# tanmayb123/OpenAI-Whisper-CoreML

Hardware: AMD Instinct MI355X
Metric: audio-sec/s (RTF) + decoder tok/s, Whisper-large-v2 30s chunks, 1->8 GPU (higher is better)
Workload: dtype bf16

## Files before the change

include/whisper_mi355x_debug.h:

```cpp
#ifndef WHISPER_MI355X_DEBUG_H
#define WHISPER_MI355X_DEBUG_H

#include "whisper_mi355x.h"

#ifdef __cplusplus
extern "C" {
#endif

WM_API int wmdbg_mel_filterbank(int n_mels, float *out);
WM_API int wmdbg_mel80(float *out);

WM_API int wmdbg_gemm(wm_ctx *ctx, const float *A, const float *W, const float *bias, float *C, int M, int N,
               int K, int epi);
WM_API int wmdbg_layernorm(wm_ctx *ctx, const float *x, const float *g, const float *b, int rows, int d,
                    float *out_f32, float *out_bf16_as_f32);
WM_API int wmdbg_enc_attention(wm_ctx *ctx, const float *q, const float *k, const float *v, int B, int H, int S,
                        float *out);
WM_API int wmdbg_dec_gemv(wm_ctx *ctx, const float *x, const float *ln_g, const float *ln_b, const float *W,
                   const float *bias, float *out, int B, int N, int K);
WM_API int wmdbg_dec_gemv_resid(wm_ctx *ctx, const float *x, const float *W, const float *bias, float *resid, float *copy_bf16,
                         float *stats, int B, int N, int K);
WM_API int wmdbg_dec_attention(wm_ctx *ctx, const float *q, const float *k, const float *v, int B, int H, int T,
                        int n_keys, int nsplit, float *out);
WM_API int wmdbg_dec_self_attention_off(wm_ctx *ctx, const float *q, const float *k, const float *v, int B, int H, int T,
                                        int pos, const int32_t *off, float *out);

WM_API int wmdbg_bench_dec_gemv(wm_ctx *ctx, int B, int N, int K, int ln, int resid, int n_mats, int iters,
                         int nw_override, float *avg_us);
WM_API int wmdbg_bench_dec_attention(wm_ctx *ctx, int B, int H, int T, int n_keys, int nsplit, int n_slices,
                              int iters, float *avg_us);

WM_API int wmdbg_bench_launch_floor(wm_ctx *ctx, int iters, int grid, float *eager_us, float *graph_us);

WM_API int wmdbg_bench_graph_branches(wm_ctx *ctx, int iters, int grid, int us_each, float *one_us, float *two_us);

WM_API int wmdbg_bench_gemm(wm_ctx *ctx, int M, int N, int K, int epi, int iters, int n_w, float *us);

WM_API int wmdbg_set_gemm_tile(int tile);

WM_API int wmdbg_lane_parts(int B, int lanes, int explicit_lanes, int n_text_state);
WM_API int wmdbg_cu_mask(int cu_lo, int cu_hi, uint32_t *mask8);

WM_API int wmdbg_set_precision(wm_ctx *ctx, int precision);

WM_API int wmdbg_set_tuning(const char *key, int value);
WM_API int wmdbg_group_count(int B, int lanes, int explicit_lanes);
WM_API int wmdbg_right_align(const int32_t *prompts, int stride, const int32_t *prompt_len, int b0, int Bg, int32_t *table_out,
                             int32_t *off_out);

WM_API int wmdbg_cand_groups(int B, int N, int lanes, int explicit_lanes, int32_t *b0_out, int32_t *cg_out);
WM_API int wmdbg_dec_attention_cand(wm_ctx *ctx, const float *q, const float *k, const float *v, int C, int N, int H, int T,
                                    int n_keys, const int32_t *live_rows, int n_live, float *out);
WM_API int wmdbg_dec_attention_cand_shared(wm_ctx *ctx, const float *q, const float *k, const float *v, int C, int N, int H,
                                           int T, int n_keys, const int32_t *live_rows, int n_live, float *out);

WM_API int wmdbg_sample_noise(wm_ctx *ctx, uint64_t seed, int chunk, int gi, int n0, int count, float *g);

WM_API int wmdbg_dtw(wm_ctx *ctx, const float *x, int B, const int32_t *N, const int32_t *M, int ld, int32_t *start_frame_out);
WM_API int wmdbg_align_capture(wm_ctx *ctx, float *matrix_out);
WM_API int wmdbg_align_matrix(wm_ctx *ctx, const float *q, const float *keys, int L, int H, int B, int Tq, int J,
                              const int32_t *hl, const int32_t *hh, int S, const int32_t *n_text, const int32_t *n_frames,
                              int medfilt_width, float qk_scale, float *x, float *col_stats);
WM_API int wmdbg_align_token_prob(wm_ctx *ctx, const float *logits, int B, int V, int ldo, const int32_t *tok, int eot,
                                  float *prob);

WM_API int wmdbg_beam_select(int N, int n_from, int32_t eot, int32_t pad, int room, const float *sum, const int32_t *list_n,
                             const int32_t *list_tok, const float *list_lp, int32_t *n_next, int32_t *src, int32_t *tok,
                             float *lp, float *new_sum, int32_t *n_fin, int32_t *fin_src, float *fin_lp, float *fin_sum);
WM_API double wmdbg_rank_score(double sum, int n_text, float length_penalty);
WM_API int wmdbg_beam_fill_order(int N, const float *sum, int32_t *order_out);
WM_API int wmdbg_beam_trace(wm_ctx *ctx, float *trace_out);
WM_API int wmdbg_beam_topk(wm_ctx *ctx, const float *logits, int rows, int V, int N, const int32_t *suppress, int n_suppress,
                           const int32_t *rng, int32_t ts_begin, int32_t *list_n, int32_t *list_tok, float *list_lp);
WM_API int wmdbg_beam_reorder(wm_ctx *ctx, uint16_t *cache, int L2, int rows, int H, int T, int N, int pos, int n_prompt,
                              const int32_t *src, const int32_t *wdone, int32_t *seq, float *logprob);

#ifdef __cplusplus
}
#endif
#endif
```

openai-whisper-coreml_amd/csrc/debug_hooks.cpp:

```cpp
#include <math.h>
#include <stdio.h>
#include <stdlib.h>
#include <string.h>

#include <algorithm>
#include <vector>

#include "../../include/whisper_mi355x_debug.h"
#include "beam.h"
#include "model.h"

int wm_gemm_set_tile_override(int tile);
extern "C" int wmdbg_set_gemm_tile(int tile) { return wm_gemm_set_tile_override(tile); }

extern "C" int wmdbg_set_tuning(const char *key, int value) {
    WM_REQUIRE(key, WM_ERR_INVALID, "wmdbg_set_tuning: null key");
    struct { const char *name; int *field; } table[] = {
        {"gemv_tn", &g_wm_tuning.gemv_tn}, {"gemv_nblk", &g_wm_tuning.gemv_nblk}, {"gemv_no_ppw2", &g_wm_tuning.gemv_no_ppw2}, {"gemv_ppw2_nblk", &g_wm_tuning.gemv_ppw2_nblk},
        {"prefetch_max_b", &g_wm_tuning.prefetch_max_b}, {"xattn_split_below", &g_wm_tuning.xattn_split_below},
        {"xattn_wgs", &g_wm_tuning.xattn_wgs}, {"xattn_no_flat", &g_wm_tuning.xattn_no_flat},
        {"xattn_lds_pad", &g_wm_tuning.xattn_lds_pad}, {"xattn_splits", &g_wm_tuning.xattn_splits},
        {"gemm_tile", &g_wm_tuning.gemm_tile}, {"gemm128_pipe", &g_wm_tuning.gemm128_pipe}, {"gemm_gm", &g_wm_tuning.gemm_gm}, {"no_early_stop", &g_wm_tuning.no_early_stop},
        {"xattn_no_deep", &g_wm_tuning.xattn_no_deep}, {"xattn_never_short", &g_wm_tuning.xattn_never_short},         {"logits_tn", &g_wm_tuning.logits_tn}, {"enc_attn_mfma_sum", &g_wm_tuning.enc_attn_mfma_sum},
        {"group_chunks", &g_wm_tuning.group_chunks}, {"argmax_rows_per_wg", &g_wm_tuning.argmax_rows_per_wg}, {"xattn_fuse_q", &g_wm_tuning.xattn_fuse_q},
        {"lane_parts", &g_wm_tuning.lane_parts}, {"lane_solo_cus", &g_wm_tuning.lane_solo_cus}, {"frontend_per_wave_twiddles", &g_wm_tuning.frontend_per_wave_twiddles},
    };
    if (strcmp(key, "reset") == 0) { g_wm_tuning = WmTuning(); return WM_OK; }
    for (auto &e : table)
        if (strcmp(key, e.name) == 0) { *e.field = value; return WM_OK; }
    wm_set_error("wmdbg_set_tuning: unknown key '%s'", key);
    return WM_ERR_INVALID;
}

extern "C" int wmdbg_group_count(int B, int lanes, int explicit_lanes) { return wm_group_count(B, lanes, explicit_lanes != 0, 0); }
extern "C" int wmdbg_cand_groups(int B, int N, int lanes, int explicit_lanes, int32_t *b0_out, int32_t *cg_out) {
    if (B < 1 || N < 1 || N > WM_MAX_BEST_OF || !b0_out || !cg_out) return -1;
    std::vector<int> b0, cg;
    const int G = wm_cand_groups(B, N, lanes, explicit_lanes != 0, b0, cg);
    for (int g = 0; g < G; ++g) { b0_out[g] = b0[g]; cg_out[g] = cg[g]; }
    return G;
}
extern "C" int wmdbg_right_align(const int32_t *prompts, int stride, const int32_t *prompt_len, int b0, int Bg,
                                 int32_t *table_out, int32_t *off_out) {
    std::vector<int32_t> table, off;
    const int P = wm_right_align(prompts, stride, prompt_len, b0, Bg, table, off);
    std::copy(table.begin(), table.end(), table_out);
    std::copy(off.begin(), off.end(), off_out);
    return P;
}
extern "C" int wmdbg_lane_parts(int B, int lanes, int explicit_lanes, int n_text_state) {
    return wm_lane_parts(B, lanes, explicit_lanes != 0, n_text_state, 0);
}
extern "C" int wmdbg_cu_mask(int cu_lo, int cu_hi, uint32_t *mask8) { return wm_cu_mask(cu_lo, cu_hi, mask8); }

extern "C" int wmdbg_mel_filterbank(int n_mels, float *out) {
    WM_REQUIRE(out && n_mels > 0 && n_mels <= 256, WM_ERR_INVALID, "bad args");
    std::vector<float> f;
    wm_mel_filterbank(n_mels, f);
    memcpy(out, f.data(), f.size() * sizeof(float));
    return WM_OK;
}
extern "C" int wmdbg_mel80(float *out) {
    WM_REQUIRE(out, WM_ERR_INVALID, "null");
    memcpy(out, wm_mel80_table(), sizeof(float) * 80 * 201);
    return WM_OK;
}

static int up(void **d, const void *h, size_t bytes, hipStream_t s) {
    WM_HIP(hipMalloc(d, bytes + 512));
    WM_HIP(hipMemsetAsync(*d, 0, bytes + 512, s));
    if (h) WM_HIP(hipMemcpyAsync(*d, h, bytes, hipMemcpyHostToDevice, s));
    return WM_OK;
}
static void to_bf16(const float *in, std::vector<bf16_t> &out, size_t n) {
    out.resize(n);
    for (size_t i = 0; i < n; ++i) {
        uint32_t u;
        memcpy(&u, &in[i], 4);
        u += 0x7fffu + ((u >> 16) & 1u);
        out[i] = (bf16_t)(u >> 16);
    }
}
static void from_bf16(const std::vector<bf16_t> &in, float *out) {
    for (size_t i = 0; i < in.size(); ++i) {
        uint32_t u = (uint32_t)in[i] << 16;
        memcpy(&out[i], &u, 4);
    }
}

extern "C" int wmdbg_gemm(wm_ctx *ctx, const float *A, const float *W, const float *bias, float *C, int M, int N,
                          int K, int epi) {
    WM_TRY(wm_ctx_make_current(ctx));
    WM_REQUIRE(epi == EPI_F32 || epi == EPI_BIAS_BF16 || epi == EPI_GELU_BF16 || epi == EPI_RESID_F32, WM_ERR_INVALID,
               "wmdbg_gemm: epilogue %d not exposed", epi);
    std::vector<bf16_t> a16, w16;
    to_bf16(A, a16, (size_t)M * K);
    to_bf16(W, w16, (size_t)N * K);
    void *dA, *dW, *dB = nullptr, *dC;
    hipStream_t s = ctx->stream;
    WM_TRY(up(&dA, a16.data(), a16.size() * 2, s));
    WM_TRY(up(&dW, w16.data(), w16.size() * 2, s));
    if (bias) WM_TRY(up(&dB, bias, (size_t)N * 4, s));
    const bool f32out = (epi == EPI_F32 || epi == EPI_RESID_F32);
    WM_TRY(up(&dC, epi == EPI_RESID_F32 ? C : nullptr, (size_t)M * N * (f32out ? 4 : 2), s));
    GemmArgs g;
    memset(&g, 0, sizeof(g));
// ... 213 lines not shown
    to_bf16(v, v16, (size_t)B * H * T * 64);
    void *dq, *dk, *dv, *dp;
    hipStream_t s = ctx->stream;
    WM_TRY(up(&dq, q, (size_t)B * H * 64 * 4, s));
    WM_TRY(up(&dk, k16.data(), k16.size() * 2, s));
    WM_TRY(up(&dv, v16.data(), v16.size() * 2, s));
    WM_TRY(up(&dp, nullptr, (size_t)B * H * WM_MAXSPLIT * 66 * 4, s));
    void *datt;
    WM_TRY(up(&datt, nullptr, ((size_t)B + 15) / 16 * 16 * H * 64 * 2, s));
    int rc = nsplit == 0 ? wm_dec_self_attention(ctx, (const float *)dq, (const bf16_t *)dk, (const bf16_t *)dv, B, H, T,
                                                 n_keys, nullptr, (bf16_t *)datt)
                         : wm_dec_attention(ctx, (const float *)dq, (const bf16_t *)dk, (const bf16_t *)dv, B, H, T, n_keys,
                                            nullptr, nsplit < 0 ? 1 : nsplit, (float *)dp, (bf16_t *)datt, nsplit < 0);
    if (rc == WM_OK) {
        const size_t Bpad = ((size_t)B + 15) / 16 * 16, dd = (size_t)H * 64;
        std::vector<bf16_t> o16(Bpad * dd), lin((size_t)B * dd);
        WM_HIP(hipMemcpyAsync(o16.data(), datt, o16.size() * 2, hipMemcpyDeviceToHost, s));
        WM_HIP(hipStreamSynchronize(s));
        for (size_t b = 0; b < (size_t)B; ++b)
            for (size_t k = 0; k < dd; ++k) lin[b * dd + k] = o16[wm_tiled_offset(b, k, dd)];
        from_bf16(lin, out);
    }
    (void)hipFree(datt);
    (void)hipFree(dq); (void)hipFree(dk); (void)hipFree(dv); (void)hipFree(dp);
    return rc;
}

static int dec_attention_cand(wm_ctx *ctx, const float *q, const float *k, const float *v, int C, int N, int H, int T, int n_keys,
                              const int32_t *live_rows, int n_live, float *out, bool short_lived) {
    WM_TRY(wm_ctx_make_current(ctx));
    WM_REQUIRE(q && k && v && out, WM_ERR_INVALID, "dec_attention_cand: null pointer");
    WM_REQUIRE(N >= 1 && N <= WM_MAX_BEST_OF && C >= 1 && C * N <= WM_DEC_MAXB && H >= 1 && H <= 255 && T >= 1 && n_keys >= 1 &&
                   n_keys <= T,
               WM_ERR_INVALID, "dec_attention_cand: bad geometry");
    const int B = C * N;
    std::vector<int32_t> live((size_t)WM_DEC_MAXB + 4, 0);
    if (live_rows) {
        WM_REQUIRE(n_live >= 0 && n_live <= B, WM_ERR_INVALID, "dec_attention_cand: n_live %d outside [0, %d]", n_live, B);
        for (int i = 0; i < n_live; ++i) {
            WM_REQUIRE(live_rows[i] >= 0 && live_rows[i] < B && (i == 0 || live_rows[i] > live_rows[i - 1]), WM_ERR_INVALID,
                       "dec_attention_cand: the live list must be ascending rows of the group");
            live[i] = live_rows[i];
        }
        live[WM_DEC_MAXB] = n_live;
    }
    std::vector<bf16_t> k16, v16;
    to_bf16(k, k16, (size_t)C * H * T * 64);
    to_bf16(v, v16, (size_t)C * H * T * 64);
    void *dq, *dk, *dv, *dp, *dl, *datt;
    hipStream_t s = ctx->stream;
    const size_t att_b = ((size_t)B + 15) / 16 * 16 * H * 64 * 2;
    WM_TRY(up(&dq, q, (size_t)B * H * 64 * 4, s));
    WM_TRY(up(&dk, k16.data(), k16.size() * 2, s));
    WM_TRY(up(&dv, v16.data(), v16.size() * 2, s));
    WM_TRY(up(&dp, nullptr, (size_t)B * H * WM_MAXSPLIT * 66 * 4, s));
    WM_TRY(up(&dl, live.data(), live.size() * 4, s));
    WM_TRY(up(&datt, nullptr, att_b, s));
    WM_HIP(hipMemsetAsync(dp, 0, (size_t)B * H * WM_MAXSPLIT * 66 * 4, s));
    WM_HIP(hipMemsetAsync(datt, 0, att_b, s));
    const int *lr = live_rows ? (const int *)dl : nullptr;
    int rc = wm_dec_attention_cand(ctx, (const float *)dq, (const bf16_t *)dk, (const bf16_t *)dv, C, N, H, T, n_keys, (float *)dp,
                                   (bf16_t *)datt, nullptr, 0, 0, lr, lr ? lr + WM_DEC_MAXB : nullptr, short_lived);
    if (rc == WM_OK) {
        const size_t Bpad = ((size_t)B + 15) / 16 * 16, dd = (size_t)H * 64;
        std::vector<bf16_t> o16(Bpad * dd), lin((size_t)B * dd);
        WM_HIP(hipMemcpyAsync(o16.data(), datt, o16.size() * 2, hipMemcpyDeviceToHost, s));
        WM_HIP(hipStreamSynchronize(s));
        for (size_t b = 0; b < (size_t)B; ++b)
            for (size_t kk = 0; kk < dd; ++kk) lin[b * dd + kk] = o16[wm_tiled_offset(b, kk, dd)];
        from_bf16(lin, out);
    }
    void *fr[] = {dq, dk, dv, dp, dl, datt};
    for (void *p : fr) (void)hipFree(p);
    return rc;
}

extern "C" int wmdbg_dec_attention_cand(wm_ctx *ctx, const float *q, const float *k, const float *v, int C, int N, int H, int T,
                                        int n_keys, const int32_t *live_rows, int n_live, float *out) {
    return dec_attention_cand(ctx, q, k, v, C, N, H, T, n_keys, live_rows, n_live, out, false);
}
extern "C" int wmdbg_dec_attention_cand_shared(wm_ctx *ctx, const float *q, const float *k, const float *v, int C, int N, int H,
                                               int T, int n_keys, const int32_t *live_rows, int n_live, float *out) {
    return dec_attention_cand(ctx, q, k, v, C, N, H, T, n_keys, live_rows, n_live, out, true);
}

extern "C" int wmdbg_dec_self_attention_off(wm_ctx *ctx, const float *q, const float *k, const float *v, int B, int H, int T,
                                            int pos, const int32_t *off, float *out) {
    WM_TRY(wm_ctx_make_current(ctx));
    WM_REQUIRE(q && k && v && off && out, WM_ERR_INVALID, "dec_self_attention_off: null pointer");
    WM_REQUIRE(B >= 1 && B <= WM_DEC_MAXB && T >= 1 && pos >= 0 && pos < T, WM_ERR_INVALID, "dec_self_attention_off: bad geometry");
    for (int b = 0; b < B; ++b)
        WM_REQUIRE(off[b] >= 0 && off[b] < T, WM_ERR_INVALID, "dec_self_attention_off: off[%d] = %d outside [0, %d)", b, off[b], T);
    std::vector<bf16_t> k16, v16;
    to_bf16(k, k16, (size_t)B * H * T * 64);
    to_bf16(v, v16, (size_t)B * H * T * 64);
    void *dq, *dk, *dv, *doff, *dpos, *datt;
    hipStream_t s = ctx->stream;
    WM_TRY(up(&dq, q, (size_t)B * H * 64 * 4, s));
    WM_TRY(up(&dk, k16.data(), k16.size() * 2, s));
    WM_TRY(up(&dv, v16.data(), v16.size() * 2, s));
    WM_TRY(up(&doff, off, (size_t)B * 4, s));
    WM_TRY(up(&dpos, &pos, 4, s));
    WM_TRY(up(&datt, nullptr, ((size_t)B + 15) / 16 * 16 * H * 64 * 2, s));
    int rc = wm_dec_self_attention(ctx, (const float *)dq, (const bf16_t *)dk, (const bf16_t *)dv, B, H, T, 0, (const int *)dpos,
                                   (bf16_t *)datt, nullptr, 0, 0, nullptr, nullptr, (const int *)doff);
    if (rc == WM_OK) {
        const size_t Bpad = ((size_t)B + 15) / 16 * 16, dd = (size_t)H * 64;
        std::vector<bf16_t> o16(Bpad * dd), lin((size_t)B * dd);
        WM_HIP(hipMemcpyAsync(o16.data(), datt, o16.size() * 2, hipMemcpyDeviceToHost, s));
        WM_HIP(hipStreamSynchronize(s));
        for (size_t b = 0; b < (size_t)B; ++b)
            for (size_t j = 0; j < dd; ++j) lin[b * dd + j] = o16[wm_tiled_offset(b, j, dd)];
        from_bf16(lin, out);
    }
    void *fr[] = {dq, dk, dv, doff, dpos, datt};
    for (void *p : fr)
        if (p) (void)hipFree(p);
    return rc;
}


extern "C" int wmdbg_bench_dec_gemv(wm_ctx *ctx, int B, int N, int K, int ln, int resid, int n_mats, int iters,
                                    int nw_override, float *avg_us) {
    (void)nw_override;
    WM_TRY(wm_ctx_make_current(ctx));
    WM_REQUIRE(B >= 1 && B <= WM_DEC_MAXB, WM_ERR_INVALID, "wmdbg_bench_dec_gemv: B out of range");
    hipStream_t s = ctx->stream;
    const int Npad = ((N + 15) / 16) * 16;
    void *dW, *dx16, *dc, *dout, *dout16;
    WM_TRY(up(&dW, nullptr, (size_t)n_mats * Npad * K * 2, s));
    WM_TRY(up(&dx16, nullptr, (size_t)WM_DEC_MAXB * K * 2, s));
    WM_TRY(up(&dc, nullptr, (size_t)Npad * 4, s));
    WM_TRY(up(&dout, nullptr, (size_t)WM_DEC_MAXB * Npad * 4, s));
    WM_TRY(up(&dout16, nullptr, (size_t)WM_DEC_MAXB * Npad * 2, s));
    WM_HIP(hipMemsetAsync(dW, 0x3c, (size_t)n_mats * Npad * K * 2, s));
    DecGemvArgs a;
    memset(&a, 0, sizeof(a));
    a.B = B; a.N = N; a.K = K; a.out_f32 = (float *)dout; a.ldo = Npad; a.epi = resid ? DE_RESID : DE_Q;
    a.a = (const bf16_t *)dx16; a.c2 = (const float *)dc;
    void *dstat;
    WM_TRY(up(&dstat, nullptr, (size_t)(WM_DEC_MAXB / 16) * 2 * (K > N ? K : N) * 4 + 4096, s));
    if (resid) { a.stats_out = (float *)dstat; a.out_bf16 = (bf16_t *)dout16; }
    if (ln) { a.c1 = (const float *)dc; a.stats_in = (const float *)dstat; a.stats_parts = K / 16; }
    hipEvent_t e0, e1;
    WM_HIP(hipEventCreate(&e0));
    WM_HIP(hipEventCreate(&e1));
    int rc = WM_OK;
    hipGraph_t g = nullptr;
    hipGraphExec_t ge = nullptr;
    WM_HIP(hipStreamBeginCapture(s, hipStreamCaptureModeThreadLocal));
    for (int i = 0; i < iters && rc == WM_OK; ++i) {
        a.W = (const bf16_t *)dW + (size_t)(i % n_mats) * Npad * K;
        rc = wm_dec_gemv(ctx, a);
    }
    WM_HIP(hipStreamEndCapture(s, &g));
    if (rc == WM_OK) {
        WM_HIP(hipGraphInstantiate(&ge, g, nullptr, nullptr, 0));
        WM_HIP(hipGraphLaunch(ge, s));
        WM_HIP(hipStreamSynchronize(s));
        WM_HIP(hipEventRecord(e0, s));
        WM_HIP(hipGraphLaunch(ge, s));
    }
    WM_HIP(hipEventRecord(e1, s));
    WM_HIP(hipStreamSynchronize(s));
    float ms = 0.f;
    WM_HIP(hipEventElapsedTime(&ms, e0, e1));
// ... 445 lines not shown
```

openai-whisper-coreml_amd/csrc/dec_kernels.hip:

```cpp
#include <stdlib.h>

#include <atomic>
#include <string.h>

#include "dec_close.h"
#include "model.h"
#include "philox.h"

namespace {

typedef __attribute__((ext_vector_type(8))) __bf16 bf16x8;
typedef __attribute__((ext_vector_type(4))) float f32x4;
typedef __attribute__((ext_vector_type(4))) unsigned u32x4;

typedef __attribute__((ext_vector_type(2))) float f32x2;
typedef __attribute__((ext_vector_type(2))) __bf16 bf16x2;

__device__ __forceinline__ unsigned pack2(float a, float b) {
    const f32x2 v = {a, b};
    return __builtin_bit_cast(unsigned, __builtin_convertvector(v, bf16x2));
}
__device__ __forceinline__ float gelu_erf(float x) {
    return 0.5f * x * (1.0f + erff(x * 0.70710678118654752440f));
}
// ... 750 lines not shown
                    vb -= (long)(ob - pos_k) * 64;
                    ob = pos_k;
                    load_block(kb, vb, 0, 0, kall[0], vall[0]);
                }
            }
        }
        int nk = n_keys;
        if constexpr (OFF) nk = pos_k + 1 - ob;
        float qe[8];
#pragma unroll
        for (int i = 0; i < 4; ++i) {
            qe[i] = q0[i] * 0.125f;
            qe[4 + i] = q1[i] * 0.125f;
        }
        float m_run = -1e30f, l_run = 0.f;
        float oa[8] = {0, 0, 0, 0, 0, 0, 0, 0};
        auto process_block = [&](int r0, const u32x4 (&kv)[U], const u32x4 (&vv)[U]) {
            attn_block<NS, U, SELF>(qe, r0, stream, rg, nk, kv, vv, m_run, l_run, oa);
        };
        if (DEEP) {
#pragma unroll
            for (int blk = 0; blk < NB; ++blk)
                if (blk * (NS * 8 * U) < nk) process_block(blk * (NS * 8 * U), kall[blk], vall[blk]);
        } else {
            if (SPEC) {
                attn_block_fence<U>(kall[0], vall[0]);
                process_block(0, kall[0], vall[0]);
            }
            for (int r0 = SPEC ? NS * 8 * U : 0; r0 < nk; r0 += NS * 8 * U) {
                u32x4 kv[U], vv[U];
                load_block(kb, vb, r0, nk - 1, kv, vv);
                attn_block_fence<U>(kv, vv);
                process_block(r0, kv, vv);
            }
        }
        attn_stream_reduce(l_run, oa);
        if (nsplit > 1) {
            if (rg == 0) {
                float *po = cold.part + ((long)bh * NS + stream) * 66;
#pragma unroll
                for (int i = 0; i < 8; ++i) po[2 + e8 * 8 + i] = oa[i];
                if (e8 == 0) {
                    po[0] = m_run;
                    po[1] = l_run;
                }
            }
            continue;
        }
        if (rg == 0) {
#pragma unroll
            for (int i = 0; i < 8; ++i) wo_[wave][e8 * 8 + i] = oa[i];
            if (e8 == 0) {
                wm_[wave] = m_run;
                wl_[wave] = l_run;
            }
        }
        __syncthreads();
        if (tid < 64)
            cold.att[wm_tiled_offset((size_t)b, (size_t)(h * 64 + tid), (size_t)d)] = f2bf(attn_merge<NS>(wm_, wl_, &wo_[0][0], 64, tid));
    }
}

template <int NS, int U, bool NT, bool DEEP = false>
__global__ __launch_bounds__(DEEP ? 256 : NS * 64) void dec_xrows_attn_kernel(
    const float *__restrict__ q, const bf16_t *__restrict__ kc, const bf16_t *__restrict__ vc,
    const int *__restrict__ pos_ptr, const int *__restrict__ live_rows ,
    unsigned packA , unsigned packB ,
    unsigned packC , AttnCold cold) {
    const int H = (int)(packA & 0xffu), nsplit = (int)((packA >> 8) & 0xffu), flat_wpw = (int)(packA >> 16);
    const int T_stride = (int)(packB & 0xffffu), n_keys_const = (int)(packB >> 16);
    int n_bh = (int)(packC & 0xffffu);
    const int n_wg = (int)(packC >> 16);
    const int d = H * 64;
    const int *n_live_ptr = live_rows ? live_rows + WM_DEC_MAXB : nullptr;
    bf16_t *att = cold.att;
    float *part = cold.part;
    const char *pf_ptr = cold.pf_ptr;
    const long pf_tile_bytes = cold.pf_tile_bytes;
    if ((int)blockIdx.x >= n_wg) {
        l2_warm_tile(pf_ptr, pf_tile_bytes, (int)blockIdx.x - n_wg, blockDim.x);
        return;
    }
    if (n_live_ptr) n_bh = *n_live_ptr * H;
    __shared__ float wm_[NS], wl_[NS];
    __shared__ float wo_[NS][64];
    const int tid = threadIdx.x, lane = tid & 63, wave = tid >> 6;
    const int rg = lane >> 3, e8 = lane & 7;
    const int n_keys = pos_ptr ? (*pos_ptr + 1) : n_keys_const;
    const int last = n_keys - 1;
    int stream = (int)blockIdx.y * (NS / nsplit) + wave;
    int bh0 = blockIdx.x, bh_step = n_wg;
    if (flat_wpw > 0) {
        const int unit = (int)blockIdx.x * flat_wpw + wave;
        if (unit >= n_bh * NS) return;
        bh0 = unit / NS;
        stream = unit % NS;
        bh_step = n_bh;
    }
    for (int pi = bh0; pi < n_bh; pi += bh_step) {
        if (flat_wpw == 0 && pi != (int)blockIdx.x) __syncthreads();
        const int h = pi % H;
        const int b = live_rows ? live_rows[pi / H] : pi / H;
        const int bh = b * H + h;
        const bf16_t *kb = kc + (long)bh * T_stride * 64 + e8 * 8;
        const bf16_t *vb = vc + (long)bh * T_stride * 64 + e8 * 8;
        float qe[8];
        {
            const float *qp = q + (long)b * d + h * 64 + e8 * 8;
#pragma unroll
            for (int i = 0; i < 8; ++i) qe[i] = qp[i] * 0.125f;
        }
        float m_run = -1e30f, l_run = 0.f;
        float oa[8] = {0, 0, 0, 0, 0, 0, 0, 0};
        auto load_block = [&](int r0, u32x4 (&kv)[U], u32x4 (&vv)[U]) {
            attn_load_block<NS, U, NT>(kb, vb, r0, stream, rg, n_keys, last, kv, vv);
        };
        auto process_block = [&](int r0, const u32x4 (&kv)[U], const u32x4 (&vv)[U]) {
            attn_block<NS, U, false>(qe, r0, stream, rg, n_keys, kv, vv, m_run, l_run, oa);
        };
        if (DEEP) {
            constexpr int NB = ATT_MAXK / (NS * 8 * U);
            u32x4 kall[NB][U], vall[NB][U];
#pragma unroll
            for (int blk = 0; blk < NB; ++blk) load_block(blk * (NS * 8 * U), kall[blk], vall[blk]);
#pragma unroll
            for (int blk = 0; blk < NB; ++blk)
                if (blk * (NS * 8 * U) < n_keys) process_block(blk * (NS * 8 * U), kall[blk], vall[blk]);
        } else {
            for (int r0 = 0; r0 < n_keys; r0 += NS * 8 * U) {
                u32x4 kv[U], vv[U];
                load_block(r0, kv, vv);
                process_block(r0, kv, vv);
            }
        }
        attn_stream_reduce(l_run, oa);
        if (nsplit > 1) {
            if (rg == 0) {
                float *po = part + ((long)bh * NS + stream) * 66;
#pragma unroll
                for (int i = 0; i < 8; ++i) po[2 + e8 * 8 + i] = oa[i];
                if (e8 == 0) {
                    po[0] = m_run;
                    po[1] = l_run;
                }
            }
            continue;
        }
        if (rg == 0) {
#pragma unroll
            for (int i = 0; i < 8; ++i) wo_[wave][e8 * 8 + i] = oa[i];
            if (e8 == 0) {
                wm_[wave] = m_run;
                wl_[wave] = l_run;
            }
        }
        __syncthreads();
        if (tid < 64)
            att[wm_tiled_offset((size_t)b, (size_t)(h * 64 + tid), (size_t)d)] = f2bf(attn_merge<NS>(wm_, wl_, &wo_[0][0], 64, tid));
    }
}

struct CandLive {
    int r_lo, r_hi;
    unsigned long long head_lo, head_hi;
};
template <int N>
__device__ __forceinline__ void cand_window(const CandLive &L, int wj, int lane, int &c, unsigned &lm) {
    const int rank_lo = (int)__builtin_amdgcn_mbcnt_hi((unsigned)(L.head_lo >> 32), __builtin_amdgcn_mbcnt_lo((unsigned)L.head_lo, 0u));
    const int rank_hi = (int)__builtin_amdgcn_mbcnt_hi((unsigned)(L.head_hi >> 32), __builtin_amdgcn_mbcnt_lo((unsigned)L.head_hi, 0u)) +
                        __popcll(L.head_lo);
    const unsigned long long sel_lo = __ballot(((L.head_lo >> lane) & 1ull) && rank_lo == wj);
    const unsigned long long sel_hi = __ballot(((L.head_hi >> lane) & 1ull) && rank_hi == wj);
    int row;
    if (sel_lo) row = __builtin_amdgcn_readlane(L.r_lo, __builtin_ctzll(sel_lo));
    else row = __builtin_amdgcn_readlane(L.r_hi, sel_hi ? __builtin_ctzll(sel_hi) : 0);
    c = row / N;
    lm = 0u;
#pragma unroll
    for (int s = 0; s < N; ++s) {
        const int r = c * N + s;
        if ((__ballot(L.r_lo == r) | __ballot(L.r_hi == r)) != 0ull) lm |= 1u << s;
    }
}

template <int N, bool NT>
__global__ __launch_bounds__(512) void dec_xcand_attn_kernel(
    const float *__restrict__ q, const bf16_t *__restrict__ kc, const bf16_t *__restrict__ vc,
    const int *__restrict__ live_rows , bf16_t *__restrict__ att,
    float *__restrict__ part, unsigned packA , unsigned packB ,
    unsigned packC , const char *pf_ptr, long pf_tile_bytes) {
    constexpr int NS = 8, U = 4;
    static_assert(N >= 1 && N <= 8, "1 .. 8 candidates per window");
    constexpr int NP = N <= 5 ? N : (N + 1) / 2;
    const int H = (int)(packA & 0xffu), flat_wpw = (int)(packA >> 16);
    const int T_stride = (int)(packB & 0xffffu), n_keys = (int)(packB >> 16);
    const int C = (int)(packC & 0xffffu), n_wg = (int)(packC >> 16);
    const int d = H * 64;
    if ((int)blockIdx.x >= n_wg) {
        l2_warm_tile(pf_ptr, pf_tile_bytes, (int)blockIdx.x - n_wg, blockDim.x);
        return;
    }
    __shared__ float wm_[N][NS], wl_[N][NS];
    __shared__ float wo_[N][NS][64];
    const int tid = threadIdx.x, lane = tid & 63, wave = tid >> 6;
    const int rg = lane >> 3, e8 = lane & 7;
    const int last = n_keys - 1;
    CandLive L;
    {
        int n_live = C * N, p_lo = lane - 1, p_hi = lane + 63;
        L.r_lo = lane;
        L.r_hi = lane + 64;
        if (live_rows) {
            n_live = live_rows[WM_DEC_MAXB];
            L.r_lo = live_rows[lane];
            L.r_hi = live_rows[lane + 64];
            p_lo = live_rows[lane > 0 ? lane - 1 : 0];
            p_hi = live_rows[lane + 63];
        }
        const bool v_lo = lane < n_live, v_hi = lane + 64 < n_live;
        L.r_lo = v_lo ? L.r_lo : -1;
        L.r_hi = v_hi ? L.r_hi : -1;
        L.head_lo = __ballot(v_lo && (lane == 0 || p_lo / N != L.r_lo / N));
        L.head_hi = __ballot(v_hi && p_hi / N != L.r_hi / N);
    }
    const int n_pairs = (__popcll(L.head_lo) + __popcll(L.head_hi)) * H;
    int stream = wave;
    int p0 = blockIdx.x, p_step = n_wg;
    if (flat_wpw > 0) {
        const int unit = (int)blockIdx.x * flat_wpw + wave;
        if (unit >= n_pairs * NS) return;
        p0 = unit / NS;
        stream = unit % NS;
        p_step = n_pairs;
    }
    for (int pi = p0; pi < n_pairs; pi += p_step) {
        if (flat_wpw == 0 && pi != (int)blockIdx.x) __syncthreads();
        const int h = pi % H;
        int c;
        unsigned lm;
        cand_window<N>(L, pi / H, lane, c, lm);
        const int ch = c * H + h;
// ... 584 lines not shown
        if (two) {
            nblk = 2;
            p.bgroups = (blocks + 1) / 2;
        }
    }
    p.n_tg = (p.n_tiles + tn - 1) / tn;
    p.n_tg_pad = p.bgroups > 1 ? (p.n_tg + 7) / 8 * 8 : p.n_tg;
    int grid = p.n_tg_pad * p.bgroups;
    if (pf_enabled(a.B) && a.pf_ptr && a.pf_rows >= 16 && grid % 8 == 0) {
        p.pf_ptr = (const char *)a.pf_ptr;
        p.pf_tile_bytes = 16L * a.pf_k * 2;
        p.pf_tiles = a.pf_rows / 16;
        p.pf_head_major = a.pf_head_major;
        grid += a.pf_head_major ? 32 * (a.pf_head_major / a.B + 2) : p.pf_tiles;
    }
    switch (a.epi * 2 + (ln ? 1 : 0)) {
        case DE_QKV * 2 + 1: {
            WmProfScope ps(&ctx->prof, "dec_gemv_ln_qkv", ctx->stream);
            return launch_gemv<DE_QKV, true>(ctx, p, spw, tn, nblk, nw, grid, ppw);
        }
        case DE_Q * 2 + 1: {
            WmProfScope ps(&ctx->prof, "dec_gemv_ln_q", ctx->stream);
            return launch_gemv<DE_Q, true>(ctx, p, spw, tn, nblk, nw, grid, ppw);
        }
        case DE_GELU * 2 + 1: {
            WmProfScope ps(&ctx->prof, "dec_gemv_ln_fc1", ctx->stream);
            return launch_gemv<DE_GELU, true>(ctx, p, spw, tn, nblk, nw, grid, ppw);
        }
        case DE_LOGITS * 2 + 1: {
            WmProfScope ps(&ctx->prof, "dec_gemv_ln_logits", ctx->stream);
            return launch_gemv<DE_LOGITS, true>(ctx, p, spw, tn, nblk, nw, grid, ppw);
        }
        case DE_LOGITS_X * 2 + 1: {
            WmProfScope ps(&ctx->prof, "dec_gemv_ln_logits_x", ctx->stream);
            return launch_gemv<DE_LOGITS_X, true>(ctx, p, spw, tn, nblk, nw, grid, ppw);
        }
        case DE_RESID * 2: {
            WmProfScope ps(&ctx->prof, a.K > a.N ? "dec_gemv_fc2" : "dec_gemv_attn_out", ctx->stream);
            return launch_gemv<DE_RESID, false>(ctx, p, spw, tn, nblk, nw, grid, ppw);
        }
        case DE_Q * 2: {
            WmProfScope ps(&ctx->prof, "dec_gemv_plain", ctx->stream);
            return launch_gemv<DE_Q, false>(ctx, p, spw, tn, nblk, nw, grid, ppw);
        }
        default:
            wm_set_error("dec_gemv: unsupported (epilogue %d, LayerNorm %d) pair", a.epi, (int)ln);
            return WM_ERR_INVALID;
    }
}

int wm_ln_fold(wm_ctx *ctx, const bf16_t *W, const float *g, const float *beta, const float *bias, int N, int K,
               bf16_t *Wf, float *c1, float *c2) {
    const int npad = (N + 15) / 16 * 16;
    ln_fold_kernel<<<npad, 256, 0, ctx->stream>>>(W, g, beta, bias, N, K, Wf, c1, c2);
    WM_HIP(hipGetLastError());
    return WM_OK;
}

int wm_dec_embed(wm_ctx *ctx, const int *seq, const int *pos_ptr, int B, const bf16_t *emb, const float *pemb,
                 int d, float *x, bf16_t *xb, float *stats_out, float *mean_buf, const int *off) {
    WmProfScope ps(&ctx->prof, "dec_embed", ctx->stream);
    dec_embed_kernel<<<B, 256, 0, ctx->stream>>>(seq, pos_ptr, B, emb, pemb, d, x, xb, stats_out, mean_buf, off);
    WM_HIP(hipGetLastError());
    return WM_OK;
}

int wm_dec_attn_splits(int B, int H) {
    const int bh = B * H;
    const int thr = g_wm_tuning.xattn_split_below;
    if (bh >= thr) return 1;
    int ns = 2;
    while (ns < 8 && bh * ns < 192) ns *= 2;
    return ns;
}

int wm_dec_attention(wm_ctx *ctx, const float *q, const bf16_t *kc, const bf16_t *vc, int B, int H,
                     int T_stride, int n_keys, const int *pos_ptr, int nsplit, float *part, bf16_t *att,
                     bool cross, const bf16_t *pf_ptr, int pf_rows, int pf_k, const int *live_rows, const int *n_live,
                     bool short_lived) {
    WM_REQUIRE(nsplit == 1 || nsplit == 2 || nsplit == 4 || nsplit == 8, WM_ERR_INVALID,
               "dec_attention: nsplit %d is not 1, 2, 4 or 8", nsplit);
    WM_REQUIRE(T_stride <= ATT_MAXK && n_keys <= ATT_MAXK, WM_ERR_INVALID,
               "dec_attention: more than %d keys", ATT_MAXK);
    WM_REQUIRE(nsplit == 1 || part != nullptr, WM_ERR_INVALID, "dec_attention: split launch without a partials buffer");
    WM_REQUIRE(H >= 1 && H <= 255 && B * H < 65536, WM_ERR_INVALID, "dec_attention: %d heads x %d rows do not fit the packed arguments", H, B);
    WM_REQUIRE((!live_rows && !n_live) || n_live == live_rows + WM_DEC_MAXB, WM_ERR_INVALID, "dec_attention: the live count must follow the live rows");
    {
        WmProfScope ps(&ctx->prof, cross ? "dec_attn_cross" : "dec_attn_self", ctx->stream);
        const int cap_cus = g_wm_tuning.xattn_wgs > 0 && g_wm_tuning.xattn_wgs < ctx->n_cus ? g_wm_tuning.xattn_wgs : ctx->n_cus;
        const int cap = short_lived ? (1 << 30) : cap_cus;
        int n_wg = B * H;
        if (n_wg > cap) {
            const int rounds = (n_wg + cap - 1) / cap;
            n_wg = (n_wg + rounds - 1) / rounds;
        }
        int gx = n_wg;
        long tile_bytes = 0;
        if (pf_enabled(B) && pf_ptr && nsplit == 1 && gx % 8 == 0 && pf_rows >= 16) {
            tile_bytes = 16L * pf_k * 2;
            gx += pf_rows / 16;
        }
        const bool no_flat = g_wm_tuning.xattn_no_flat != 0;
        if (nsplit > 1 && !no_flat) {
            const int units = B * H * 8;
            int wpw = (units + 255) / 256;
            wpw = wpw < 1 ? 1 : (wpw > 4 ? 4 : wpw);
            const int g = (units + wpw - 1) / wpw;
            const AttnCold cold = {att, part, nullptr, 0};
            const unsigned pA = (unsigned)H | (8u << 8) | ((unsigned)wpw << 16), pB = (unsigned)T_stride | ((unsigned)n_keys << 16);
            const unsigned pC = (unsigned)(B * H) | ((unsigned)g << 16);
            WM_REQUIRE(g < 65536, WM_ERR_INVALID, "dec_attention: flat grid too large");
            if (g_wm_tuning.xattn_no_deep)
                dec_xrows_attn_kernel<8, 4, WM_XATTN_NT><<<g, wpw * 64, 0, ctx->stream>>>(
                    q, kc, vc, pos_ptr, live_rows, pA, pB, pC, cold);
            else if ((size_t)B * H * T_stride * 64 * 2 * 2 <= (size_t)3200 * 1024)
                dec_rows_attn_kernel<8, 4, false, true><<<g, wpw * 64, 0, ctx->stream>>>(
                    q, kc, vc, pos_ptr, live_rows, pA, pB, pC, cold);
            else
                dec_rows_attn_kernel<8, 4, WM_XATTN_NT, true><<<g, wpw * 64, 0, ctx->stream>>>(
                    q, kc, vc, pos_ptr, live_rows, pA, pB, pC, cold);
        } else {
            dim3 grid(gx, nsplit);
            const int lds_pad = g_wm_tuning.xattn_lds_pad;
            static std::atomic<int> pad_set[64];
            if (lds_pad > pad_set[ctx->device & 63].load(std::memory_order_acquire)) {
                WM_HIP(hipFuncSetAttribute((const void *)dec_xrows_attn_kernel<8, 4, WM_XATTN_NT>,
                                           hipFuncAttributeMaxDynamicSharedMemorySize, lds_pad));
                pad_set[ctx->device & 63].store(lds_pad, std::memory_order_release);
            }
            const AttnCold cold = {att, part, (const char *)pf_ptr, tile_bytes};
            const unsigned pA = (unsigned)H | ((unsigned)nsplit << 8), pB = (unsigned)T_stride | ((unsigned)n_keys << 16);
            const unsigned pC = (unsigned)(B * H) | ((unsigned)n_wg << 16);
            dec_xrows_attn_kernel<8, 4, WM_XATTN_NT><<<grid, (8 / nsplit) * 64, nsplit == 1 ? lds_pad : 0, ctx->stream>>>(
                q, kc, vc, pos_ptr, live_rows, pA, pB, pC, cold);
        }
        WM_HIP(hipGetLastError());
    }
    if (nsplit > 1) {
        WmProfScope ps(&ctx->prof, "dec_attn_combine", ctx->stream);
        dec_attn_combine_kernel<8><<<B * H, 64, 0, ctx->stream>>>(part, H, H * 64, att);
        WM_HIP(hipGetLastError());
    }
    return WM_OK;
}

namespace {
template <int N>
int launch_xcand(wm_ctx *ctx, const float *q, const bf16_t *kc, const bf16_t *vc, int C, int H, int T_stride, int n_keys,
                 float *part, bf16_t *att, const bf16_t *pf_ptr, int pf_rows, int pf_k, const int *live_rows, bool short_lived,
                 bool *flat) {
    const int pairs = C * H;
    *flat = pairs < 256 && !short_lived;
    const unsigned pB = (unsigned)T_stride | ((unsigned)n_keys << 16);
    long tile_bytes = 0;
    int warm = 0;
    if (pf_enabled(C * N) && pf_ptr && pf_rows >= 16) {
        tile_bytes = 16L * pf_k * 2;
        warm = pf_rows / 16;
    }
    if (*flat) {
        const int units = pairs * 8;
        int wpw = (units + 255) / 256;
        wpw = wpw < 1 ? 1 : (wpw > 8 ? 8 : wpw);
        const int g = (units + wpw - 1) / wpw;
        if (g % 8 != 0) warm = 0;
        const unsigned pA = (unsigned)H | ((unsigned)wpw << 16), pC = (unsigned)C | ((unsigned)g << 16);
        dec_xcand_attn_kernel<N, WM_XATTN_NT><<<g + warm, wpw * 64, 0, ctx->stream>>>(
            q, kc, vc, live_rows, att, part, pA, pB, pC, warm ? (const char *)pf_ptr : nullptr, warm ? tile_bytes : 0);
        WM_HIP(hipGetLastError());
        return WM_OK;
    }
    const int cap_cus = g_wm_tuning.xattn_wgs > 0 && g_wm_tuning.xattn_wgs < ctx->n_cus ? g_wm_tuning.xattn_wgs : ctx->n_cus;
    const int cap = short_lived ? (1 << 30) : cap_cus;
    int n_wg = pairs;
    if (n_wg > cap) {
        const int rounds = (n_wg + cap - 1) / cap;
// ... 250 lines not shown
```

openai-whisper-coreml_amd/csrc/wm_internal.h:

```cpp
#pragma once
#include <hip/hip_runtime.h>
#include <stdint.h>
#include <exception>
#include <map>
#include <new>
#include <string>
#include <vector>

#include "../../include/whisper_mi355x.h"

void wm_set_error(const char *fmt, ...);

#define WM_HIP(expr)                                                                      \
    do {                                                                                  \
        hipError_t _e = (expr);                                                           \
        if (_e != hipSuccess) {                                                           \
            wm_set_error("%s:%d: %s failed: %s", __FILE__, __LINE__, #expr,               \
                         hipGetErrorString(_e));                                          \
            return WM_ERR_HIP;                                                            \
        }                                                                                 \
    } while (0)

#define WM_TRY(expr)                                                                      \
    do {                                                                                  \
// ... 66 lines not shown
struct WmFrontend {
    float *cos32 = nullptr, *sin32 = nullptr, *win32 = nullptr;
    double *cos64 = nullptr, *sin64 = nullptr, *win64 = nullptr;
    int *band_start[2] = {nullptr, nullptr};
    int *band_len[2] = {nullptr, nullptr};
    float *band_w[2] = {nullptr, nullptr};
    int band_maxw[2] = {0, 0};
    void *gmax = nullptr;
    int gmax_cap = 0;
    void *scratch = nullptr;
    size_t scratch_bytes = 0;
    void *long_tab = nullptr;
    size_t long_tab_bytes = 0;
    bool ready = false;
};

struct WmLongRec {
    long long base;
    long long out;
    int len;
    int T;
};
struct WmLongTab {
    const WmLongRec *rec;
    const int2 *blk;
};

int wm_frontend_init(WmFrontend *fe, hipStream_t stream);
void wm_frontend_destroy(WmFrontend *fe);
int wm_frontend_run(WmFrontend *fe, WmProfiler *prof, hipStream_t stream, const void *d_pcm,
                    wm_dtype pcm_dtype, int n_chunks, int n_mels, void *d_out,
                    wm_dtype out_dtype);
int wm_frontend_run_long(WmFrontend *fe, WmProfiler *prof, hipStream_t stream, const void *d_pcm, wm_dtype pcm_dtype,
                         const int64_t *offs, int R, int n_mels, float *d_out);
inline int64_t wm_long_frames(int64_t len) { return (len + WM_N_SAMPLES) / WM_HOP; }
void wm_mel_filterbank(int n_mels, std::vector<float> &out );
const float *wm_mel80_table();

struct WmModel;
struct wm_ctx;

struct WmDebugHooks {
    int (*encode_dev)(wm_ctx *ctx, const float *d_mel, int B, float *d_xa);
    int (*decode_logits_dev)(wm_ctx *ctx, const int32_t *host_tokens , int B, int T, const float *d_xa,
                             float *d_logits );
};

struct wm_ctx {
    int device = 0;
    hipStream_t stream = nullptr;
    WmProfiler prof;
    WmFrontend fe;
    WmModel *model = nullptr;
    float stage_ms[3] = {0, 0, 0};
    std::vector<wm_ctx *> lanes;
    const WmDebugHooks *dbg_hooks = nullptr;
    int max_lanes = 0;
    int n_cus = 256, cu_lo = 0, cu_hi = 32;
    std::vector<wm_ctx *> part_lanes[2];
    bool no_cu_masks = false;
    std::map<int, wm_ctx *> solo_lanes;
};
template <typename F>
int wm_for_each_lane(wm_ctx *ctx, bool with_self, F &&fn) {
    if (with_self) WM_TRY(fn(ctx));
    for (wm_ctx *lane : ctx->lanes) WM_TRY(fn(lane));
    for (auto &v : ctx->part_lanes)
        for (wm_ctx *lane : v) WM_TRY(fn(lane));
    for (auto &kv : ctx->solo_lanes) WM_TRY(fn(kv.second));
    return WM_OK;
}
int wm_clone_cus(wm_ctx *parent, int cu_lo, int cu_hi, wm_ctx **out);
int wm_cu_mask(int cu_lo, int cu_hi, uint32_t mask[8]);

int wm_ctx_make_current(const wm_ctx *ctx);
int wm_group_count(int B, int L, bool explicit_lanes, int gc_probe);
int wm_cand_groups(int B, int N, int L, bool explicit_lanes, std::vector<int> &b0, std::vector<int> &cg);
void wm_balanced_cut(int B, int G, std::vector<int> &b0, std::vector<int> &cg);
int wm_right_align(const int32_t *prompts, int stride, const int32_t *prompt_len, int b0, int Bg, std::vector<int32_t> &table,
                   std::vector<int32_t> &off);
double wm_rank_score(double sum, int n_text, float length_penalty);
int wm_lane_parts(int B, int L, bool explicit_lanes, int n_text_state, int n_text_layer);

struct WmTuning {
    int gemv_tn = 0;
    int gemv_nblk = 0;
    int gemv_ppw2_nblk = 0;
    int gemv_no_ppw2 = 0;
    int prefetch_max_b = 16;
    int xattn_split_below = 96;
    int xattn_wgs = 256;
    int xattn_no_flat = 0;
    int xattn_lds_pad = 84 * 1024;
    int xattn_splits = 0;
    int gemm_tile = 0;
    int gemm_gm = 4;
    int gemm128_pipe = 0;
    int no_early_stop = 0;
    int logits_tn = 0;
    int enc_attn_mfma_sum = 0;
    int xattn_never_short = 0;
    int xattn_no_deep = 0;
    int xattn_fuse_q = 1;
    int argmax_rows_per_wg = 0;
    int group_chunks = 0;
    int frontend_per_wave_twiddles = 0;
    int lane_parts = 0;
    int lane_solo_cus = 0;
};
extern WmTuning g_wm_tuning;

#include <atomic>
extern std::atomic<int> g_wm_active_decodes[64];
```

Measured before the change: 2236.

## Prefetch next head pair's query and first KV block in decoder attention loop

```diff
diff --git a/include/whisper_mi355x_debug.h b/include/whisper_mi355x_debug.h
--- a/include/whisper_mi355x_debug.h
+++ b/include/whisper_mi355x_debug.h
@@ -53,6 +53,8 @@
                                     int n_keys, const int32_t *live_rows, int n_live, float *out);
 WM_API int wmdbg_dec_attention_cand_shared(wm_ctx *ctx, const float *q, const float *k, const float *v, int C, int N, int H,
                                            int T, int n_keys, const int32_t *live_rows, int n_live, float *out);
+WM_API int wmdbg_dec_attention_shape(wm_ctx *ctx, const float *q, const float *k, const float *v, int B, int H, int T,
+                                     int n_keys, int shape, int arg, const int32_t *live_rows, int n_live, float *out);
 
 WM_API int wmdbg_sample_noise(wm_ctx *ctx, uint64_t seed, int chunk, int gi, int n0, int count, float *g);
 
diff --git a/openai-whisper-coreml_amd/csrc/debug_hooks.cpp b/openai-whisper-coreml_amd/csrc/debug_hooks.cpp
--- a/openai-whisper-coreml_amd/csrc/debug_hooks.cpp
+++ b/openai-whisper-coreml_amd/csrc/debug_hooks.cpp
@@ -21,7 +21,7 @@
         {"xattn_wgs", &g_wm_tuning.xattn_wgs}, {"xattn_no_flat", &g_wm_tuning.xattn_no_flat},
         {"xattn_lds_pad", &g_wm_tuning.xattn_lds_pad}, {"xattn_splits", &g_wm_tuning.xattn_splits},
         {"gemm_tile", &g_wm_tuning.gemm_tile}, {"gemm128_pipe", &g_wm_tuning.gemm128_pipe}, {"gemm_gm", &g_wm_tuning.gemm_gm}, {"no_early_stop", &g_wm_tuning.no_early_stop},
-        {"xattn_no_deep", &g_wm_tuning.xattn_no_deep}, {"xattn_never_short", &g_wm_tuning.xattn_never_short},         {"logits_tn", &g_wm_tuning.logits_tn}, {"enc_attn_mfma_sum", &g_wm_tuning.enc_attn_mfma_sum},
+        {"xattn_no_deep", &g_wm_tuning.xattn_no_deep}, {"xattn_short_pairs", &g_wm_tuning.xattn_short_pairs}, {"xattn_never_short", &g_wm_tuning.xattn_never_short},         {"logits_tn", &g_wm_tuning.logits_tn}, {"enc_attn_mfma_sum", &g_wm_tuning.enc_attn_mfma_sum},
         {"group_chunks", &g_wm_tuning.group_chunks}, {"argmax_rows_per_wg", &g_wm_tuning.argmax_rows_per_wg}, {"xattn_fuse_q", &g_wm_tuning.xattn_fuse_q},
         {"lane_parts", &g_wm_tuning.lane_parts}, {"lane_solo_cus", &g_wm_tuning.lane_solo_cus}, {"frontend_per_wave_twiddles", &g_wm_tuning.frontend_per_wave_twiddles},
     };
@@ -401,6 +401,56 @@
 extern "C" int wmdbg_dec_attention_cand_shared(wm_ctx *ctx, const float *q, const float *k, const float *v, int C, int N, int H,
                                                int T, int n_keys, const int32_t *live_rows, int n_live, float *out) {
     return dec_attention_cand(ctx, q, k, v, C, N, H, T, n_keys, live_rows, n_live, out, true);
+}
+
+extern "C" int wmdbg_dec_attention_shape(wm_ctx *ctx, const float *q, const float *k, const float *v, int B, int H, int T,
+                                         int n_keys, int shape, int arg, const int32_t *live_rows, int n_live, float *out) {
+    WM_TRY(wm_ctx_make_current(ctx));
+    WM_REQUIRE(q && k && v && out, WM_ERR_INVALID, "dec_attention_shape: null pointer");
+    WM_REQUIRE(B >= 1 && B <= WM_DEC_MAXB && H >= 1 && H <= 255 && T >= 1 && n_keys >= 1 && n_keys <= T, WM_ERR_INVALID,
+               "dec_attention_shape: bad geometry");
+    WM_REQUIRE(shape >= 0 && shape <= 2 && arg >= 1, WM_ERR_INVALID, "dec_attention_shape: shape %d / %d", shape, arg);
+    std::vector<int32_t> live((size_t)WM_DEC_MAXB + 4, 0);
+    if (live_rows) {
+        WM_REQUIRE(n_live >= 0 && n_live <= B, WM_ERR_INVALID, "dec_attention_shape: n_live %d outside [0, %d]", n_live, B);
+        for (int i = 0; i < n_live; ++i) {
+            WM_REQUIRE(live_rows[i] >= 0 && live_rows[i] < B, WM_ERR_INVALID, "dec_attention_shape: live row outside the group");
+            live[i] = live_rows[i];
+        }
+        live[WM_DEC_MAXB] = n_live;
+    }
+    std::vector<bf16_t> k16, v16;
+    to_bf16(k, k16, (size_t)B * H * T * 64);
+    to_bf16(v, v16, (size_t)B * H * T * 64);
+    void *dq, *dk, *dv, *dp, *dl, *datt;
+    hipStream_t s = ctx->stream;
+    const size_t att_b = ((size_t)B + 15) / 16 * 16 * H * 64 * 2;
+    WM_TRY(up(&dq, q, (size_t)B * H * 64 * 4, s));
+    WM_TRY(up(&dk, k16.data(), k16.size() * 2, s));
+    WM_TRY(up(&dv, v16.data(), v16.size() * 2, s));
+    WM_TRY(up(&dp, nullptr, (size_t)B * H * WM_MAXSPLIT * 66 * 4, s));
+    WM_TRY(up(&dl, live.data(), live.size() * 4, s));
+    WM_TRY(up(&datt, nullptr, att_b, s));
+    const int *lr = live_rows ? (const int *)dl : nullptr;
+    const WmTuning saved = g_wm_tuning;
+    if (shape == 0) g_wm_tuning.xattn_wgs = arg;
+    if (shape == 1) g_wm_tuning.xattn_short_pairs = arg;
+    int rc = wm_dec_attention(ctx, (const float *)dq, (const bf16_t *)dk, (const bf16_t *)dv, B, H, T, n_keys, nullptr,
+                              shape == 2 ? arg : 1, (float *)dp, (bf16_t *)datt, true, nullptr, 0, 0, lr,
+                              lr ? lr + WM_DEC_MAXB : nullptr, shape == 1);
+    g_wm_tuning = saved;
+    if (rc == WM_OK) {
+        const size_t Bpad = ((size_t)B + 15) / 16 * 16, dd = (size_t)H * 64;
+        std::vector<bf16_t> o16(Bpad * dd), lin((size_t)B * dd);
+        WM_HIP(hipMemcpyAsync(o16.data(), datt, o16.size() * 2, hipMemcpyDeviceToHost, s));
+        WM_HIP(hipStreamSynchronize(s));
+        for (size_t b = 0; b < (size_t)B; ++b)
+            for (size_t kk = 0; kk < dd; ++kk) lin[b * dd + kk] = o16[wm_tiled_offset(b, kk, dd)];
+        from_bf16(lin, out);
+    }
+    void *fr[] = {dq, dk, dv, dp, dl, datt};
+    for (void *p : fr) (void)hipFree(p);
+    return rc;
 }
 
 extern "C" int wmdbg_dec_self_attention_off(wm_ctx *ctx, const float *q, const float *k, const float *v, int B, int H, int T,
diff --git a/openai-whisper-coreml_amd/csrc/dec_kernels.hip b/openai-whisper-coreml_amd/csrc/dec_kernels.hip
--- a/openai-whisper-coreml_amd/csrc/dec_kernels.hip
+++ b/openai-whisper-coreml_amd/csrc/dec_kernels.hip
@@ -856,8 +856,8 @@
         return;
     }
     if (n_live_ptr) n_bh = *n_live_ptr * H;
-    __shared__ float wm_[NS], wl_[NS];
-    __shared__ float wo_[NS][64];
+    __shared__ float wm_[2][NS], wl_[2][NS];
+    __shared__ float wo_[2][NS][64];
     const int tid = threadIdx.x, lane = tid & 63, wave = tid >> 6;
     const int rg = lane >> 3, e8 = lane & 7;
     const int n_keys = pos_ptr ? (*pos_ptr + 1) : n_keys_const;
@@ -871,19 +871,32 @@
         stream = unit % NS;
         bh_step = n_bh;
     }
+    int b = 0, h = 0;
+    const bf16_t *kb = kc, *vb = vc;
+    float qr[8];
+    u32x4 kp[U], vp[U];
+    auto pair_row = [&](int p) { return live_rows ? live_rows[p / H] : p / H; };
+    int row_ahead = 0;
+    auto request_pair = [&](int p, int row) {
+        h = p % H;
+        b = row;
+        row_ahead = p + bh_step < n_bh ? pair_row(p + bh_step) : 0;
+        const int bh = b * H + h;
+        kb = kc + (long)bh * T_stride * 64 + e8 * 8;
+        vb = vc + (long)bh * T_stride * 64 + e8 * 8;
+        const float *qp = q + (long)b * d + h * 64 + e8 * 8;
+#pragma unroll
+        for (int i = 0; i < 8; ++i) qr[i] = qp[i];
+        if (!DEEP) attn_load_block<NS, U, NT>(kb, vb, 0, stream, rg, n_keys, last, kp, vp);
+    };
+    if (bh0 < n_bh) request_pair(bh0, pair_row(bh0));
+    int slot = 0;
     for (int pi = bh0; pi < n_bh; pi += bh_step) {
-        if (flat_wpw == 0 && pi != (int)blockIdx.x) __syncthreads();
-        const int h = pi % H;
-        const int b = live_rows ? live_rows[pi / H] : pi / H;
-        const int bh = b * H + h;
-        const bf16_t *kb = kc + (long)bh * T_stride * 64 + e8 * 8;
-        const bf16_t *vb = vc + (long)bh * T_stride * 64 + e8 * 8;
+        const int b_cur = b, h_cur = h;
+        const int pn = pi + bh_step;
         float qe[8];
-        {
-            const float *qp = q + (long)b * d + h * 64 + e8 * 8;
-#pragma unroll
-            for (int i = 0; i < 8; ++i) qe[i] = qp[i] * 0.125f;
-        }
+#pragma unroll
+        for (int i = 0; i < 8; ++i) qe[i] = qr[i] * 0.125f;
         float m_run = -1e30f, l_run = 0.f;
         float oa[8] = {0, 0, 0, 0, 0, 0, 0, 0};
         auto load_block = [&](int r0, u32x4 (&kv)[U], u32x4 (&vv)[U]) {
@@ -901,16 +914,28 @@
             for (int blk = 0; blk < NB; ++blk)
                 if (blk * (NS * 8 * U) < n_keys) process_block(blk * (NS * 8 * U), kall[blk], vall[blk]);
         } else {
-            for (int r0 = 0; r0 < n_keys; r0 += NS * 8 * U) {
+            process_block(0, kp, vp);
+            int r1 = NS * 8 * U;
+            asm volatile("" : "+s"(r1));
+            for (int r0 = r1; r0 < n_keys; r0 += NS * 8 * U) {
                 u32x4 kv[U], vv[U];
                 load_block(r0, kv, vv);
+                __builtin_amdgcn_sched_barrier(0);
                 process_block(r0, kv, vv);
             }
+        }
+        if (pn < n_bh) {
+            request_pair(pn, row_ahead);
+        } else {
+#pragma unroll
+            for (int i = 0; i < 8; ++i) qr[i] = 0.f;
+#pragma unroll
+            for (int u = 0; u < U; ++u) kp[u] = vp[u] = u32x4{0u, 0u, 0u, 0u};
         }
         attn_stream_reduce(l_run, oa);
         if (nsplit > 1) {
             if (rg == 0) {
-                float *po = part + ((long)bh * NS + stream) * 66;
+                float *po = part + ((long)(b_cur * H + h_cur) * NS + stream) * 66;
 #pragma unroll
                 for (int i = 0; i < 8; ++i) po[2 + e8 * 8 + i] = oa[i];
                 if (e8 == 0) {
@@ -922,15 +947,17 @@
         }
         if (rg == 0) {
 #pragma unroll
-            for (int i = 0; i < 8; ++i) wo_[wave][e8 * 8 + i] = oa[i];
+            for (int i = 0; i < 8; ++i) wo_[slot][wave][e8 * 8 + i] = oa[i];
             if (e8 == 0) {
-                wm_[wave] = m_run;
-                wl_[wave] = l_run;
+                wm_[slot][wave] = m_run;
+                wl_[slot][wave] = l_run;
             }
         }
         __syncthreads();
         if (tid < 64)
-            att[wm_tiled_offset((size_t)b, (size_t)(h * 64 + tid), (size_t)d)] = f2bf(attn_merge<NS>(wm_, wl_, &wo_[0][0], 64, tid));
+            att[wm_tiled_offset((size_t)b_cur, (size_t)(h_cur * 64 + tid), (size_t)d)] =
+                f2bf(attn_merge<NS>(wm_[slot], wl_[slot], &wo_[slot][0][0], 64, tid));
+        slot ^= 1;
     }
 }
 
@@ -1681,16 +1708,19 @@
                "dec_attention: nsplit %d is not 1, 2, 4 or 8", nsplit);
     WM_REQUIRE(T_stride <= ATT_MAXK && n_keys <= ATT_MAXK, WM_ERR_INVALID,
                "dec_attention: more than %d keys", ATT_MAXK);
+    WM_REQUIRE(T_stride >= 1 && (pos_ptr || n_keys >= 1), WM_ERR_INVALID, "dec_attention: no keys");
     WM_REQUIRE(nsplit == 1 || part != nullptr, WM_ERR_INVALID, "dec_attention: split launch without a partials buffer");
     WM_REQUIRE(H >= 1 && H <= 255 && B * H < 65536, WM_ERR_INVALID, "dec_attention: %d heads x %d rows do not fit the packed arguments", H, B);
     WM_REQUIRE((!live_rows && !n_live) || n_live == live_rows + WM_DEC_MAXB, WM_ERR_INVALID, "dec_attention: the live count must follow the live rows");
     {
         WmProfScope ps(&ctx->prof, cross ? "dec_attn_cross" : "dec_attn_self", ctx->stream);
         const int cap_cus = g_wm_tuning.xattn_wgs > 0 && g_wm_tuning.xattn_wgs < ctx->n_cus ? g_wm_tuning.xattn_wgs : ctx->n_cus;
-        const int cap = short_lived ? (1 << 30) : cap_cus;
         int n_wg = B * H;
-        if (n_wg > cap) {
-            const int rounds = (n_wg + cap - 1) / cap;
+        if (short_lived) {
+            const int k = g_wm_tuning.xattn_short_pairs > 0 ? g_wm_tuning.xattn_short_pairs : 1;
+            n_wg = (n_wg + k - 1) / k;
+        } else if (n_wg > cap_cus) {
+            const int rounds = (n_wg + cap_cus - 1) / cap_cus;
             n_wg = (n_wg + rounds - 1) / rounds;
         }
         int gx = n_wg;
diff --git a/openai-whisper-coreml_amd/csrc/wm_internal.h b/openai-whisper-coreml_amd/csrc/wm_internal.h
--- a/openai-whisper-coreml_amd/csrc/wm_internal.h
+++ b/openai-whisper-coreml_amd/csrc/wm_internal.h
@@ -172,6 +172,7 @@
 double wm_rank_score(double sum, int n_text, float length_penalty);
 int wm_lane_parts(int B, int L, bool explicit_lanes, int n_text_state, int n_text_layer);
 
+constexpr int WM_XATTN_SHORT_PAIRS = 1;
 struct WmTuning {
     int gemv_tn = 0;
     int gemv_nblk = 0;
@@ -190,6 +191,7 @@
     int logits_tn = 0;
     int enc_attn_mfma_sum = 0;
     int xattn_never_short = 0;
+    int xattn_short_pairs = WM_XATTN_SHORT_PAIRS;
     int xattn_no_deep = 0;
     int xattn_fuse_q = 1;
     int argmax_rows_per_wg = 0;
```

Measured after the change: 2258 (median of 3 runs). Within noise of the previous version (+1.0%).
